# insitro/FastVim

Hardware: AMD Instinct MI355X
Metric: images/sec FastVim-T 224px bs=128/GPU fwd+bwd (+all-reduce +AdamW +EMA), whole job (higher is better)
Workload: dtype bf16; 1 GPU; FastVim-T 224x224 bs=128/GPU bf16 training step, synthetic ImageNet tensors (BASELINE configs[1]); global_batch=128, parallelism=dp1, hip_graph=True, optimizer_in_step=True, final_loss_hex=0x1.779ca20000000p+0

## Files before the change

fastvim_amd/_lib.py:

```python
import ctypes
import os
import threading

import torch

_PKG = os.path.dirname(os.path.abspath(__file__))
LIB_PATH = os.path.join(_PKG, "libfastvim_hip.so")

FV_F32, FV_BF16, FV_F16 = 0, 1, 2
_DTYPES = {torch.float32: FV_F32, torch.bfloat16: FV_BF16, torch.float16: FV_F16}

_lib = None

C_ABI_SYMBOLS = (
    "fv_last_error", "fv_version",
    "fv_selective_scan_fwd", "fv_selective_scan_bwd_workspace", "fv_selective_scan_bwd",
    "fv_causal_conv1d_fwd", "fv_causal_conv1d_bwd", "fv_scan_expand_skip_fwd",
    "fv_mixer_conv_pool_fwd", "fv_mixer_scan_fwd", "fv_mixer_xproj_scan_fwd_ok", "fv_mixer_xproj_scan_fwd", "fv_mixer_combine_fwd",
    "fv_mixer_bwd_blocks", "fv_mixer_combine_bwd", "fv_mixer_scan_bwd_chunks", "fv_mixer_scan_bwd_chunks_b",
    "fv_mixer_scan_bwd_ckpt_floats", "fv_mixer_scan_bwd_partials", "fv_mixer_scan_bwd", "fv_mixer_scan_bwd_dir", "fv_mixer_scan_bwd_ckpt", "fv_mixer_scan_bwd_segments", "fv_mixer_scan_bwd_seg_floats", "fv_mixer_scan_bwd_seg_partials", "fv_mixer_scan_bwd_seg_chunks", "fv_mixer_scan_bwd_seg", "fv_mixer_scan_fwd_ckpt", "fv_mixer_scan_ckpt_floats", "fv_mixer_scan_fwd_segments", "fv_mixer_scan_fwd_seg_floats", "fv_mixer_scan_fwd_seg", "fv_rows_segment_sum", "fv_rows_gather", "fv_mixer_conv_pool_bwd", "fv_mixer_conv_pool_bwd2_ok", "fv_mixer_conv_pool_bwd2", "fv_mixer_scan_bwd_xproj_ok", "fv_mixer_scan_bwd_xproj", "fv_chunk_rows_bf16", "fv_reduce_partials", "fv_reduce_partials_multi",
    "fv_add_norm_blocks", "fv_add_norm_fwd", "fv_add_norm_bwd", "fv_gemm_bf16", "fv_gemm_bf16_tn_grouped", "fv_gemm_bf16_tn_grouped_ld", "fv_mixer_xproj_fwd", "fv_mixer_xproj_bwd_slices", "fv_mixer_xproj_bwd", "fv_mixer_xproj_bwd2", "fv_mixer_xproj_bwd3_ok", "fv_mixer_xproj_bwd3", "fv_adamw_flat", "fv_soft_target_ce",
    "fv_patch_unfold", "fv_gemm_bf16_rowbias", "fv_mean_pool_fwd", "fv_mean_pool_bwd", "fv_droppath_table", "fv_scale_cast",
    "fv_column_sum", "fv_gemm_bf16_addnorm", "fv_gemm_bf16_dgrad_addnorm_blocks", "fv_gemm_bf16_dgrad_addnorm_bwd", "fv_gemm_bf16_dgrad_addnorm_bwd2", "fv_gemm_bf16_addnorm2", "fv_mixer_combine_out_proj_addnorm_ok", "fv_mixer_combine_out_proj_addnorm", "fv_gemm_f32",
    "fv_mixer_conv_pool_bwd_dgrad_ok", "fv_mixer_conv_pool_bwd_dgrad_blocks", "fv_mixer_conv_pool_bwd_dgrad", "fv_transpose_bf16_batched", "fv_gemm_bf16_tn_grouped_wide8",
# ... 5 lines not shown
    "fv_patch_unfold_chan", "fv_chan_embed_table", "fv_chan_embed_scatter",
    "fv_mixer_plan",
    "fv_bn1d_stats", "fv_bn1d_apply", "fv_bn1d_bwd", "fv_sgd_flat", "fv_lars_partials_per_segment", "fv_lars_sumsq_partials", "fv_lars_flat",
    "fv_tap_ln_blocks", "fv_tap_ln_fwd", "fv_tap_ln_bwd", "fv_ln2d_blocks", "fv_ln2d_fwd", "fv_ln2d_bwd",
    "fv_swap_params_ema", "fv_eval_accumulate",
    "fv_patch_unfold_u8", "fv_patch_unfold_mix_u8", "fv_patch_unfold_chan_u8",
    "fv_random_erase", "fv_patch_unfold_u8_re", "fv_patch_unfold_mix_u8_re",
    "fv_mae_loss_ok", "fv_mae_loss_fwd", "fv_mae_loss_bwd",
    "fv_mae_mask_plan", "fv_tokens_gather", "fv_mae_decoder_tokens_fwd", "fv_mae_decoder_tokens_bwd",
    "fv_resample_u8_ok", "fv_resample_workspace_ints", "fv_resample_coeffs", "fv_resample_u8",
    "fv_randaug_ok", "fv_randaug_workspace_bytes", "fv_randaug_stats", "fv_randaug_apply",
    "fv_jpeg_probe", "fv_jpeg_entropy_decode", "fv_jpeg_table_ints", "fv_jpeg_idct", "fv_jpeg_rgb",
    "fv_jpeg_packed_bound", "fv_jpeg_entropy_decode_packed", "fv_jpeg_idct_packed",
    "fv_mae_noise", "fv_mae_mask_plan_keyed",
    "fv_jpeg_index_bound", "fv_jpeg_build_index", "fv_jpeg_index_stage", "fv_jpeg_stream_table_ints", "fv_jpeg_huff",
)


_tls = threading.local()


class _DeviceGuarded:

    def __init__(self, cdll):
        self._cdll = cdll
        self._wrapped = {}

    def __getattr__(self, name):
        w = self._wrapped.get(name)
        if w is None:
# ... 73 lines not shown
```

fastvim_amd/csrc/gemm_mfma.hip:

```cpp
#include <stdlib.h>
#include <utility>

#include "common.h"
#include "gemm_tiles.h"

namespace {


#ifdef FASTVIM_TUNING_HOOKS
unsigned long long* g_fv_stamps = nullptr;
__device__ __forceinline__ void fv_stamp(unsigned long long* buf, int slot) {
  if (buf && threadIdx.x == 0) {
    unsigned long long t;
    __builtin_amdgcn_sched_barrier(0);
    asm volatile("s_memtime %0\n\ts_waitcnt lgkmcnt(0)" : "=s"(t)::"memory");
    __builtin_amdgcn_sched_barrier(0);
    buf[(size_t)blockIdx.x * 8 + slot] = t;
  }
}
#define FV_STAMP(ne, slot) fv_stamp((ne)->stamps, slot)
#else
#define FV_STAMP(ne, slot) ((void)0)
#endif

// ... 46 lines not shown
  const int tiles_n = (p.N + BN - 1) / BN, tiles_m = (p.M + BM - 1) / BM;
  const int nblk = NORM_EPI != 0 ? (int)gridDim.x : tiles_m * tiles_n;
  int bid = block_id;
  if constexpr (XREMAP) {
    const int q8 = nblk / 8, r8 = nblk % 8, xcd = bid % 8, j = bid / 8;
    bid = (xcd < r8 ? xcd * (q8 + 1) : r8 * (q8 + 1) + (xcd - r8) * q8) + j;
  }
  const int tm = bid / tiles_n, tn = bid % tiles_n;
  const int rpt = (NORM_EPI != 0 && ne->rpt > 0) ? ne->rpt : BM;
  const int m0 = tm * rpt, n0 = tn * BN;
  const int mlim = NORM_EPI != 0 ? min(p.M, m0 + rpt) : p.M;
  const int kbeg = split * p.k_per_split;
  const int kend = min(p.K, kbeg + p.k_per_split);
  const int nt = (kend - kbeg + BK - 1) / BK;

  if constexpr (NORM_EPI != 0) FV_STAMP(ne, 0);
  f32x4 acc[NB][MB];
#pragma unroll
  for (int a = 0; a < NB; ++a)
#pragma unroll
    for (int b = 0; b < MB; ++b) acc[a][b] = (f32x4){0.f, 0.f, 0.f, 0.f};
  constexpr bool NE_PRE = NORM_EPI != 0 && BM <= 64;
  constexpr int NE_IT = NE_PRE ? BM / 4 / 8 : 1;
  float4 ne_r[NE_IT][2][3];
  float4 ne_g[NORM_EPI == 2 ? NE_IT : 1][2][3];
  if constexpr (NORM_EPI == 2 && NE_PRE) {
    const int lr = lane % 16, gr = lane / 16;
#pragma unroll
    for (int it = 0; it < NE_IT; ++it)
#pragma unroll
      for (int u = 0; u < 2; ++u) {
        const int row = m0 + wv * (BM / 4) + it * 8 + u * 4 + gr, rowc = row < p.M ? row : p.M - 1;
#pragma unroll
        for (int k = 0; k < 3; ++k)
          ne_g[it][u][k] = ne->dres_out ? *reinterpret_cast<const float4*>(ne->dres_out + (size_t)rowc * BN + (k * 16 + lr) * 4)
                                        : make_float4(0.f, 0.f, 0.f, 0.f);
      }
  }
  if constexpr (NE_PRE) {
    const int lr = lane % 16, gr = lane / 16;
#pragma unroll
// ... 26 lines not shown
        if constexpr (OPA) fa[i] = ka.get(ks, i);
        else fa[i] = frag<AMODE, BM>(sA(cur), wm * MB + i, ks, lane);
      }
#pragma unroll
      for (int i = 0; i < NB; ++i) {
        if constexpr (OPB) fb[i] = kb.get(ks, i);
        else fb[i] = frag<BMODE, BN>(sB(cur), wn * NB + i, ks, lane);
      }
#pragma unroll
      for (int a = 0; a < NB; ++a)
#pragma unroll
        for (int b = 0; b < MB; ++b)
          acc[a][b] = __builtin_amdgcn_mfma_f32_16x16x32_bf16(fb[a], fa[b], acc[a][b], 0, 0, 0);
    }
  };
  if constexpr (GLDS) {
    GldsPlan<AMODE, BM, NT> ga;
    GldsPlan<BMODE, BN, NT> gb;
    ga.init(p.A, p.lda, m0, p.M, tid);
    gb.init(p.B, p.ldb, n0, p.N, tid);
    ga.issue(sA(0), kbeg, tid);
    gb.issue(sB(0), kbeg, tid);
    __syncthreads();
    if constexpr (NORM_EPI != 0) FV_STAMP(ne, 1);
    for (int t = 0; t < nt; ++t) {
      const int cur = t & 1;
#ifdef FASTVIM_TUNING_HOOKS
      if (t + 1 < nt && dbg != 2) {
        ga.issue(sA(cur ^ 1), kbeg + (dbg == 3 ? 0 : (t + 1) * BK), tid);
        gb.issue(sB(cur ^ 1), kbeg + (dbg == 3 ? 0 : (t + 1) * BK), tid);
      }
// ... 31 lines not shown
  }
  if constexpr (NORM_EPI != 0) FV_STAMP(ne, 2);
  const long zoff = (long)split * p.c_split_stride;
  if (p.bias && p.rb_period <= 0) {
#pragma unroll
    for (int a = 0; a < NB; ++a) {
      const int n = n0 + wn * WNC + a * 16 + (lane >> 4) * 4;
#pragma unroll
      for (int j = 0; j < 4; ++j) {
        const float bj = (n + j < p.N) ? p.bias[n + j] : 0.f;
#pragma unroll
        for (int b = 0; b < MB; ++b) acc[a][b][j] += bj;
      }
    }
  }
  if constexpr (NORM_EPI == 2) {
    static_assert(BN == 192 && WM * WN == 4 && BM % 32 == 0, "whole 192-wide rows, four waves");
    constexpr int RSB = BN * 2 + 16, LPR = 16, RPW = 4, RU = 2, RW = BM / 4;
    __syncthreads();
#pragma unroll
    for (int b = 0; b < MB; ++b)
#pragma unroll
      for (int a = 0; a < NB; ++a) {
        const f32x4 v = acc[a][b];
        uint2 pk = {pack_bf16x2(v[0], v[1]), pack_bf16x2(v[2], v[3])};
        *reinterpret_cast<uint2*>(smem + (wm * WMR + b * 16 + (lane & 15)) * RSB + (wn * WNC + a * 16 + (lane >> 4) * 4) * 2) = pk;
      }
    __syncthreads();
    FV_STAMP(ne, 3);
    const int lr = lane % LPR, gr = lane / LPR;
    const float inv_n = 1.f / (float)BN;
    float w[3][4], aw[3][4];
#pragma unroll
    for (int k = 0; k < 3; ++k) {
      const float4 t = *reinterpret_cast<const float4*>(ne->w + (k * LPR + lr) * 4);
      w[k][0] = t.x; w[k][1] = t.y; w[k][2] = t.z; w[k][3] = t.w;
#pragma unroll
      for (int e = 0; e < 4; ++e) aw[k][e] = 0.f;
    }
#pragma unroll
    for (int it = 0; it < RW / (RPW * RU); ++it) {
#pragma unroll
      for (int u = 0; u < RU; ++u) {
        const int rl = wv * RW + it * (RPW * RU) + u * RPW + gr;
        const int row = m0 + rl;
        const bool live = row < mlim;
        const int rowc = live ? row : p.M - 1;
        const size_t base = (size_t)rowc * BN;
        const float rstd = ne->rstd[rowc];
        const float sc = ne->row_scale ? ne->row_scale[rowc / ne->rows_per_scale] : 1.f;
        const float lv = live ? 1.f : 0.f;
        float xh[3][4], dxh[3][4];
        float c2 = 0.f;
#pragma unroll
        for (int k = 0; k < 3; ++k) {
          const int c = (k * LPR + lr) * 4;
          const uint2 xb = *reinterpret_cast<const uint2*>(smem + rl * RSB + c * 2);
          const float dyv[4] = {__uint_as_float(xb.x << 16), __uint_as_float(xb.x & 0xffff0000u),
                                __uint_as_float(xb.y << 16), __uint_as_float(xb.y & 0xffff0000u)};
          float4 rr4;
          if constexpr (NE_PRE) rr4 = ne_r[it][u][k];
          else rr4 = *reinterpret_cast<const float4*>(ne->residual + base + c);
          const float rr[4] = {rr4.x, rr4.y, rr4.z, rr4.w};
#pragma unroll
          for (int e = 0; e < 4; ++e) {
            const float dyl = dyv[e] * lv;
            xh[k][e] = (rr[e] - 0.f) * rstd;
            dxh[k][e] = dyl * w[k][e];
            aw[k][e] = fmaf(dyl, xh[k][e], aw[k][e]);
            c2 = fmaf(dxh[k][e], xh[k][e], c2);
          }
        }
#define FV_DPP_ADD(ctrl) c2 += __int_as_float(__builtin_amdgcn_update_dpp(0, __float_as_int(c2), ctrl, 0xf, 0xf, true))
        FV_DPP_ADD(0xB1);
        FV_DPP_ADD(0x4E);
        FV_DPP_ADD(0x141);
        FV_DPP_ADD(0x140);
#undef FV_DPP_ADD
        c2 = c2 * inv_n;
        const float c1 = 0.f;
#pragma unroll
        for (int k = 0; k < 3; ++k) {
          const int c = (k * LPR + lr) * 4;
          float4 g4;
// ... 9 lines not shown
#pragma unroll
              for (int e = 0; e < 4; ++e) dr[e] *= sc;
            uint2 pk = {pack_bf16x2(dr[0], dr[1]), pack_bf16x2(dr[2], dr[3])};
            *reinterpret_cast<uint2*>(ne->y + base + c) = pk;
            *reinterpret_cast<uint2*>(smem + rl * RSB + c * 2) = pk;
          } else {
            *reinterpret_cast<uint2*>(smem + rl * RSB + c * 2) = make_uint2(0u, 0u);
          }
        }
      }
    }
    __syncthreads();
    FV_STAMP(ne, 4);
    float* s_acc = reinterpret_cast<float*>(smem + BM * RSB);
#pragma unroll
    for (int k = 0; k < 3; ++k)
#pragma unroll
      for (int e = 0; e < 4; ++e) {
        float v = aw[k][e];
        auto r1 = __builtin_amdgcn_permlane16_swap(__float_as_uint(v), __float_as_uint(v), false, false);
        v = __uint_as_float(r1[0]) + __uint_as_float(r1[1]);
        auto r2 = __builtin_amdgcn_permlane32_swap(__float_as_uint(v), __float_as_uint(v), false, false);
        v = __uint_as_float(r2[0]) + __uint_as_float(r2[1]);
        if (gr == 0) s_acc[wv * BN + (k * LPR + lr) * 4 + e] = v;
      }
    __syncthreads();
    float* dst = ne->pw + (size_t)block_id * BN;
    for (int c = tid; c < BN; c += NT) dst[c] = (s_acc[c] + s_acc[BN + c]) + (s_acc[2 * BN + c] + s_acc[3 * BN + c]);
    FV_STAMP(ne, 5);
    if (ne->W2) {
      __syncthreads();
      constexpr int O_B = (BM * RSB + 255) / 256 * 256, O_S = O_B + 2 * 128 * BK * 2;
      tile_times_w2<BM, RSB, KS>(smem, smem + O_B, smem + O_S, ne->W2, ne->ldw2, ne->N2, ne->C2, m0, mlim, tid);
    }
    FV_STAMP(ne, 6);
    return;
  }
  if constexpr (NORM_EPI == 1) {
    static_assert(BN == 192 && WM * WN == 4 && BM % 32 == 0, "whole 192-wide rows, four waves");
    constexpr int RSB = BN * 2 + 16, LPR = 16, RPW = 4, RU = 2, RW = BM / 4;
    __syncthreads();
#pragma unroll
    for (int b = 0; b < MB; ++b)
// ... 148 lines not shown
}

template <int AMODE, int BMODE, int WM, int WN, bool GLDS, int NB = 4, int MB = 4>
__global__ __launch_bounds__(64 * WM * WN, 2) void gemm_bf16_kernel(GemmParams p) {
  gemm_bf16_body<AMODE, BMODE, WM, WN, GLDS, NB, MB>(p, blockIdx.x, blockIdx.z);
}

template <int BMROWS>
__global__ __launch_bounds__(256, 2) void gemm_addnorm_kernel(GemmParams p, NormEpi ne) {
  gemm_bf16_body<KC, KC, 2, 2, true, 6, BMROWS / 32, true, 1>(p, blockIdx.x, 0, &ne);
}

template <int BMROWS>
__global__ __launch_bounds__(256, 2) void gemm_dgrad_addnorm_bwd_kernel(GemmParams p, NormEpi ne) {
  gemm_bf16_body<KC, KS, 2, 2, true, 6, BMROWS / 32, true, 2>(p, blockIdx.x, 0, &ne);
}

template <int NV_>
__device__ __forceinline__ void wait_vmc() { asm volatile("s_waitcnt vmcnt(%0)" ::"n"(NV_) : "memory"); }
template <int OFF>
__device__ __forceinline__ u32x4 ds_read_b128_imm(uint32_t a) {
  u32x4 v;
  asm volatile("ds_read_b128 %0, %1 offset:%2" : "=v"(v) : "v"(a), "n"(OFF));
  return v;
}

template <int AMODE, int BMODE, bool CF32, bool PERSIST = false>
__device__ __forceinline__ void p256_body(const GemmParams& p, int bid, int split, char* smem, int bid_stride = 0,
                                          int bid_end = 0) {
  constexpr int HALF = 128 * BK * 2;
// ... 777 lines not shown
    constexpr size_t s1 = (size_t)2 * (BMR + 192) * BK * 2;
    constexpr size_t s2 = ((size_t)BMR * 400 + 255) / 256 * 256 + 2 * 128 * BK * 2 + 4 * 32 * 144;
    const size_t smem = s1 > s2 ? s1 : s2;
    static FvOncePerDevice attr_set;   
    if (attr_set.first()) {
      (void)hipFuncSetAttribute((const void*)gemm_dgrad_addnorm_bwd_kernel<BMR>, hipFuncAttributeMaxDynamicSharedMemorySize, (int)smem);
      (void)0;         
    }
    hipLaunchKernelGGL((gemm_dgrad_addnorm_bwd_kernel<BMR>), dim3(fv_cdiv(M, ne.rpt)), dim3(256), smem, (hipStream_t)stream, p, ne);
  };
  go(std::integral_constant<int, 64>{});
  FV_LAUNCH_CHECK();
  return FV_OK;
}

extern "C" int fv_gemm_bf16_tn_grouped_wide8(int M, int N, int Kd) {
  static const int wide8 = fv_tune("FASTVIM_WGRAD_WIDE8", 1);
  if (!wide8 || Kd < 50000) return 0;
  if (M % 256 == 0 && N % 192 == 0 && N % 256 != 0 && (long)M * N >= 1024 * 384) return 4;
  if (M % 192 == 0 && N % 256 == 0 && M % 256 != 0 && (long)M * N >= 384 * 768) return 5;
  return 0;
}

extern "C" int fv_gemm_bf16_tn_grouped(const void* const* x, const void* const* y, float* const* parts, const int* Kd,
                                       const int* M, const int* N, const int* splits, int count, fv_stream_t stream) {
  return fv_gemm_bf16_tn_grouped_ld(x, y, parts, Kd, M, N, nullptr, nullptr, splits, count, stream);
}

extern "C" int fv_gemm_bf16_tn_grouped_ld(const void* const* x, const void* const* y, float* const* parts,
                                          const int* Kd, const int* M, const int* N, const int* ldx, const int* ldy,
// ... 139 lines not shown
```

fastvim_amd/fastvim.py:

```python
import math
from functools import partial
from typing import Optional

import torch
import torch.nn as nn
import torch.nn.functional as F
from torch import Tensor

from .dense_ops import tap_layer_norm_nchw
from .layernorm import RMSNorm, layer_norm_fn, rms_norm_fn
from .linear_probe import is_probe_head, probe_head_forward
from . import glue_ops as G
from . import pixels
from . import mamba_simple_faster as msf
from .mamba_simple_faster import (ChainedBlockFn, LinearFn, Mamba, OutProjAddNormFn, _compute_dtype, _direct_grad, _shadow,
                                  linear_dgrad, linear_wgrad, out_proj_add_norm_ok)
from .mixer_ops import reduce_partials


class _EmbedEpilogueFn(torch.autograd.Function):

    @staticmethod
    def forward(ctx, lin, bias, pos):
        ctx.lin_dtype = lin.dtype
        ctx.has = (bias is not None, pos is not None)
        pb = bias.float() if bias is not None else None
        if pos is not None:
            pb = pos.float() if pb is None else pos.float() + pb
        if pb is None:
            return lin.float()
        return torch.add(pb, lin)
# ... 394 lines not shown
        return x, (H, W)

    def _chainable(self, hidden_states, lo, hi, inference_params, out_indices, carried=False):
        if inference_params is not None or out_indices is not None or hi - lo < (1 if carried else 2) or not hidden_states.is_cuda:
            return False
        if _compute_dtype(hidden_states) != torch.bfloat16 or self.embed_dim != 192:
            return False
        for blk in self.layers[lo:hi]:
            mx = blk.mixer
            if (type(blk) is not Block or type(mx) is not Mamba or not blk.fused_add_norm or not blk.residual_in_fp32
                    or not isinstance(blk.norm, RMSNorm) or blk.norm.bias is not None or mx.init_layer_scale is not None
                    or mx.out_proj.bias is not None or mx.out_proj.weight.shape[1] % 64 or mx.d_conv != 4 or mx.d_state != 16):
                return False
        return True

    def _run_layers_chained(self, hidden_states, residual, lo, hi, pend=None, close=True):
        cdt = _compute_dtype(hidden_states if pend is None else pend[0])
        pack = None
        for layer_idx in range(lo, hi):
            blk = self.layers[layer_idx]
            scale = None
            if residual is not None and isinstance(blk.drop_path, DropPath):
                scale = blk.drop_path.row_scale(hidden_states if pend is None else pend[0])
            rot = blk.rotate_every_block is True and blk.layer_idx % 2 != 0
            if pend is not None and out_proj_add_norm_ok(pend[0], pend[1], residual, blk.norm.weight, cdt):
                ChainedBlockFn.pending_in = pack
                ChainedBlockFn.defer = msf.COMBINE_IN_OUT_PROJ and torch._C._autograd._top_saved_tensors_default_hooks(True) is None
                ChainedBlockFn.pending_out = None
                try:
                    g, residual = ChainedBlockFn.apply(pend[0], pend[1], residual, blk.norm.weight, float(blk.norm.eps), scale,
                                                       *blk.mixer.mixer_fn_args(cdt, rot, defer_out_proj=True))
# ... 2 lines not shown
                    raise
                finally:
                    ChainedBlockFn.pending_in, ChainedBlockFn.defer = None, False
                pack, ChainedBlockFn.pending_out = ChainedBlockFn.pending_out, None
                pend = (g, blk.mixer.out_proj.weight)
                continue
            else:
                msf.resolve_combine(pack)
                pack = None
                if pend is not None:
                    hidden_states = LinearFn.apply(pend[0], pend[1], cdt)
                hidden_states, residual = layer_norm_fn(
                    hidden_states, blk.norm.weight, blk.norm.bias, residual=residual, eps=blk.norm.eps, prenorm=True,
                    residual_in_fp32=blk.residual_in_fp32, is_rms_norm=True, row_scale=scale, out_dtype=cdt)
            pend = (blk.mixer(hidden_states, transposed_grid=rot, defer_out_proj=True), blk.mixer.out_proj.weight)
        msf.resolve_combine(pack)
        if not close:
            return None, residual, pend
        return LinearFn.apply(pend[0], pend[1], cdt), residual

    def _run_layers_open(self, hidden_states, residual, lo, hi, pend=None):
        probe = hidden_states if pend is None else pend[0]
        if self._chainable(probe, lo, hi, None, None, carried=True):
            return self._run_layers_chained(hidden_states, residual, lo, hi, pend=pend, close=False)
        if pend is not None:
            hidden_states = self._close_run(pend)
        hidden_states, residual = self._run_layers(hidden_states, residual, lo, hi)
        return hidden_states, residual, None

    def _close_run(self, pend):
        return LinearFn.apply(pend[0], pend[1], _compute_dtype(pend[0]))

    def _run_layers(self, hidden_states, residual, lo, hi, inference_params=None, out_indices=None, outs=None):
        if self._chainable(hidden_states, lo, hi, inference_params, out_indices):
            return self._run_layers_chained(hidden_states, residual, lo, hi)
        for layer_idx in range(lo, hi):
            hidden_states, residual = self.layers[layer_idx](hidden_states, residual, inference_params=inference_params)
            if out_indices is not None and layer_idx in out_indices:
                outs.append(hidden_states)
        return hidden_states, residual

    def _final(self, hidden_states, residual):
        is_rms = isinstance(self.norm_f, RMSNorm)
        if not self.fused_add_norm:
            residual = hidden_states if residual is None else residual + self.drop_path(hidden_states)
            hidden_states = layer_norm_fn(residual.to(self.norm_f.weight.dtype), self.norm_f.weight, self.norm_f.bias,
# ... 15 lines not shown

    def _head(self, x):
        if isinstance(self.head, nn.Linear) and x.is_cuda:
            x = LinearFn.apply(x, self.head.weight, _compute_dtype(x), self.head.bias)
        elif is_probe_head(self.head) and x.is_cuda:
            x = probe_head_forward(self.head, x)
        else:
            x = self.head(x)
        if self.final_pool_type == "max":
            x = x.max(dim=1)[0]
        return x

    def forward_features(self, x, inference_params=None, out_indices=None):
        hidden_states, (H, W) = self._embed(x)
        outs = []
        hidden_states, residual = self._run_layers(hidden_states, None, 0, len(self.layers), inference_params,
                                                   out_indices, outs)
        if out_indices is not None:
            assert len(outs) == len(out_indices)
            return outs, (H, W)
        return self._final(hidden_states, residual)

    def forward(self, x, return_features=False, inference_params=None):
        half = msf.half_io(x) or self.pos_embed_dtype_is_half()
        x = self.forward_features(x, inference_params)
        if not return_features:
            x = self._head(x)
        return x.to(torch.float16) if half and torch.is_tensor(x) and x.is_floating_point() else x

    def pos_embed_dtype_is_half(self):
# ... 127 lines not shown
```

fastvim_amd/mamba_simple_faster.py:

```python
import ctypes
import math

import torch
import torch.nn as nn
import torch.nn.functional as F

from . import _lib as L
from . import mixer_ops as M
from .gemm import gemm_any_bnn, gemm_any_btn, gemm_any_nn, gemm_any_nt, gemm_any_tn, gemm_nn, gemm_nt, gemm_tn


def _shadow(w, cdt):
    sh = getattr(w, "_fv_shadow", None)
    if sh is not None and sh.dtype == cdt:
        if w._version != w._fv_shadow_version:
            with torch.no_grad():
                sh.copy_(w)
            w._fv_shadow_version = w._version
        return sh
    return w.to(cdt)


def _shadow_t(w, cdt):
    wt = getattr(w, "_fv_shadow_t", None)
# ... 278 lines not shown
                dw = M.reduce_partials(pw, nb).to(ctx.w_param.dtype)
            g2 = g.view(Mrows, d_in)
            dg = linear_dgrad(dx, _shadow(W_out, cdt)).view(B, Ltok, d_in)
            dW_out = _SideStream.run(lambda: linear_wgrad(dx, g2, W_out), dx, g)
        return dg, dW_out, dres_in.view(B, Ltok, d), dw, None, None, None


class _Ctx:

    def save_for_backward(self, *tensors):
        self.saved_tensors = tensors


COMBINE_IN_OUT_PROJ = True
CONV_IN_DGRAD = True
XPROJ_TWO_ADDENDS = True


def resolve_combine(pack):
    if pack is not None:
        M.combine_fwd(pack["xz"], pack["skip"], pack["yc"], pack["ln_w"], pack["ln_b"], pack["eps"], pack["rows"],
                      pack["cols"], pack["transposed"], out=pack["out"])


def _out_proj_add_norm_fwd(g, W_out, residual, norm_w, eps, row_scale, cdt, W_in=None, pack=None):
    B, Ltok, d_in = g.shape
    d = W_out.shape[0]
    Mrows = B * Ltok
    g2 = g.view(Mrows, d_in)
    res2 = residual.reshape(Mrows, d).contiguous()
# ... 126 lines not shown
            gd = _direct_grad(ctx.w_param)
            if gd is not None:
                M.reduce_partials(out["pw"], out["nb"], out=gd.view(-1), accumulate=True)
                dw = None
            else:
                dw = M.reduce_partials(out["pw"], out["nb"]).to(ctx.w_param.dtype)
            dx = out["dx"]
            d_in = g_prev.shape[2]
            g2 = g_prev.view(Mrows, d_in)
            dg_prev = out["dg_prev"] if out["dg_prev"] is not None else linear_dgrad(dx, _shadow(W_out_prev, cdt))
            dg_prev = dg_prev.view(B, Ltok, d_in)
            dW_out = _SideStream.run(lambda: linear_wgrad(dx, g2, W_out_prev), dx, g_prev)
        return (dg_prev, dW_out, out["dres_in"].view(B, Ltok, d), dw, None, None) + tuple(grads[1:1 + ctx.n_mixer_args])


def out_proj_add_norm_ok(g, W_out, residual, norm_w, cdt):
    return (g.is_cuda and cdt == torch.bfloat16 and g.dtype == torch.bfloat16 and g.is_contiguous()
            and W_out.shape[0] == 192 and W_out.shape[1] % 64 == 0 and residual is not None
            and residual.dtype == torch.float32 and norm_w.dtype == torch.float32)


def _compute_dtype(t):
    if torch.is_autocast_enabled():
        dt = torch.get_autocast_dtype('cuda')
        return torch.float32 if dt == torch.float16 else dt
    return torch.float32 if t.dtype == torch.float16 else t.dtype


def half_io(t):
    if torch.is_autocast_enabled():
# ... 298 lines not shown
```

fastvim_amd/mixer_ops.py:

```python
import ctypes

import torch

from . import _lib as L

f32 = ctypes.c_float


def _geo(rows, cols, transposed):
    return (1, rows) if transposed else (cols, 1)


def conv_pool_fwd(xz, conv_w, conv_b, conv_w_b, conv_b_b, rows, cols, transposed, pool_max, scaling, tpp=1,
                  D=None, D_b=None):
    B, Ltok, two_d = xz.shape
    d_in = two_d // 2
    s_i, s_j = _geo(rows, cols, transposed)
    xc = torch.empty(2, B, rows * tpp, d_in, device=xz.device, dtype=xz.dtype)
    skip = torch.empty(B, Ltok, d_in, device=xz.device, dtype=xz.dtype) if D is not None else None
    amax = torch.empty_like(xc) if pool_max else None
    rc = L.lib().fv_mixer_conv_pool_fwd(
        L.ptr(xz), L.ptr(conv_w), L.ptr(conv_b), L.ptr(conv_w_b), L.ptr(conv_b_b), L.ptr(D), L.ptr(D_b), L.ptr(xc),
        L.ptr(skip), L.ptr(amax), L.i32(B), L.i32(rows), L.i32(cols), L.i32(s_i), L.i32(s_j), L.i32(tpp), L.i32(d_in),
        L.i32(conv_w.shape[-1]), L.i32(pool_max), f32(scaling), L.i32(L.dtype_code(xz.dtype)), L.stream_of(xz))
# ... 143 lines not shown
    n = part.numel() // n_partials
    assert out.numel() == n and out.is_contiguous() and out.dtype == torch.float32
    rc = L.lib().fv_reduce_partials(L.ptr(part), L.ptr(out), L.i32(n_partials), ctypes.c_size_t(n),
                                    L.i32(accumulate), L.stream_of(part))
    L.check(rc, "reduce_partials")
    return out


def combine_out_proj_addnorm_ok(xz, rows, cols, tpp, d_model):
    B, Ltok, two_d = xz.shape
    return bool(xz.dtype == torch.bfloat16 and xz.is_contiguous() and
                L.lib().fv_mixer_combine_out_proj_addnorm_ok(L.i32(B), L.i32(rows), L.i32(cols), L.i32(tpp), L.i32(two_d // 2),
                                                             L.i32(d_model), L.i32(L.FV_BF16)))


def combine_out_proj_addnorm(xz, skip, yc, ln_w, ln_b, ln_eps, rows, cols, transposed, out, W_out_c, residual2, norm_w32,
                             row_scale, rows_per_scale, eps, W_out_pk=None):
    B, Ltok, two_d = xz.shape
    d = W_out_c.shape[0]
    Mrows = B * Ltok
    s_i, s_j = _geo(rows, cols, transposed)
    g, mean, rstd_ln = out
    y = torch.empty(Mrows, d, device=xz.device, dtype=torch.bfloat16)
    res_out = torch.empty(Mrows, d, device=xz.device, dtype=torch.float32)
    rstd = torch.empty(Mrows, device=xz.device, dtype=torch.float32)
    if W_out_pk is not None:
        assert W_out_pk.dtype == torch.bfloat16 and W_out_pk.is_contiguous() and W_out_pk.numel() == d * (two_d // 2)
        fn, W_arg, ldw = L.lib().fv_mixer_combine_out_proj_addnorm_pk, W_out_pk, two_d // 2
    else:
        fn, W_arg, ldw = L.lib().fv_mixer_combine_out_proj_addnorm, W_out_c, W_out_c.stride(0)
    rc = fn(
        L.ptr(xz), L.ptr(skip), L.ptr(yc), L.ptr(ln_w), L.ptr(ln_b), f32(ln_eps), L.ptr(g), L.ptr(mean), L.ptr(rstd_ln),
# ... 169 lines not shown
    rc = fn(
        L.ptr(xz), L.ptr(d_o), L.ptr(dxc), L.ptr(dxc2), L.ptr(conv_w), L.ptr(conv_b), L.ptr(conv_w_b), L.ptr(conv_b_b),
        L.ptr(D), L.ptr(D_b), L.ptr(dxz), L.ptr(part), L.i32(B), L.i32(rows), L.i32(cols), L.i32(s_i), L.i32(s_j),
        f32(scaling), L.ptr(W_arg), ctypes.c_long(ldwt), L.ptr(dres_out), L.ptr(r), L.ptr(rstd), L.ptr(norm_w32),
        L.ptr(row_scale), L.i32(rows_per_scale), L.ptr(dx), L.ptr(dres_in), L.ptr(pw), L.ptr(W2_arg), L.ptr(dg_prev), L.i32(N2),
        ctypes.c_long(ldw2), L.stream_of(xz))
    L.check(rc, "mixer_conv_pool_bwd_dgrad")
    if conv_grad_out is not None:
        reduce_partials(part, nb, out=conv_grad_out, accumulate=True)
        p2 = None
    else:
        p2 = reduce_partials(part, nb)
    return p2, dx, dres_in, pw, nb, dg_prev


def transpose_bf16_batched(srcs, dsts):
    lib = L.lib()
    rows, cols = srcs[0].shape
    for lo in range(0, len(srcs), 64):
        a, b = srcs[lo:lo + 64], dsts[lo:lo + 64]
        assert all(t.dtype == torch.bfloat16 and t.is_contiguous() and tuple(t.shape) == (rows, cols) for t in a)
        assert all(t.dtype == torch.bfloat16 and t.is_contiguous() and tuple(t.shape) == (cols, rows) for t in b)
        k = len(a)
        ins = (ctypes.c_void_p * k)(*[t.data_ptr() for t in a])
        outs = (ctypes.c_void_p * k)(*[t.data_ptr() for t in b])
        L.check(lib.fv_transpose_bf16_batched(ins, outs, L.i32(k), L.i32(rows), L.i32(cols), L.stream_of(a[0])), "transpose_bf16_batched")


PACK_ROWS = 192

# ... 198 lines not shown
```

include/fastvim_hip.h:

```cpp
#ifndef FASTVIM_HIP_H
#define FASTVIM_HIP_H

#include <stddef.h>
#include <stdint.h>

#ifdef __cplusplus
extern "C" {
#endif

typedef void* fv_stream_t;

enum { FV_F32 = 0, FV_BF16 = 1, FV_F16 = 2 };
enum { FV_OK = 0, FV_ERR_INVALID = -1, FV_ERR_HIP = -2, FV_ERR_UNSUPPORTED = -3 };

const char* fv_last_error(void);
#define FV_ABI_VERSION 3
int fv_version(void);

int fv_selective_scan_fwd(const void* u, const void* delta, const float* A, const void* B,
                          const void* C, const float* D, const void* z, const float* delta_bias,
                          void* out, float* last_state, int batch, int dim, int seqlen, int dstate,
                          int n_groups, int B_variable, int C_variable, int delta_softplus,
                          int dtype, fv_stream_t stream);

// ... 152 lines not shown
int fv_gemm_bf16_addnorm(const void* A, const void* W, const float* residual, const float* norm_weight,
                         const float* row_scale, int rows_per_scale, void* y, float* residual_out, float* rstd, int M,
                         int N, int K, long lda, long ldw, float eps, fv_stream_t stream);

int fv_gemm_bf16_dgrad_addnorm_blocks(int M);
int fv_gemm_bf16_dgrad_addnorm_bwd(const void* A, const void* W, const float* dresidual_out, const float* r,
                                   const float* rstd, const float* norm_weight, const float* row_scale,
                                   int rows_per_scale, void* dx, float* dresidual_in, float* partial_dw, int M, int N,
                                   int K, long lda, long ldw, fv_stream_t stream);

int fv_gemm_bf16_dgrad_addnorm_bwd2(const void* A, const void* W, const float* dresidual_out, const float* r,
                                    const float* rstd, const float* norm_weight, const float* row_scale,
                                    int rows_per_scale, void* dx, float* dresidual_in, float* partial_dw, int M, int N,
                                    int K, long lda, long ldw, const void* W2, void* C2, int N2, long ldw2,
                                    fv_stream_t stream);

int fv_mixer_combine_out_proj_addnorm_ok(int batch, int rows, int cols, int tokens_per_patch, int d_inner, int d_model,
                                         int dtype);
int fv_mixer_combine_out_proj_addnorm(const void* xz, const void* skip, const float* yc, const float* ln_w,
                                      const float* ln_b, float ln_eps, void* g, float* mean, float* rstd_ln, int batch,
                                      int rows, int cols, int tok_stride_row, int tok_stride_col, const void* W, long ldw,
                                      const float* residual, const float* norm_weight, const float* row_scale,
                                      int rows_per_scale, void* y, float* residual_out, float* rstd, float eps,
                                      fv_stream_t stream);
int fv_mixer_combine_out_proj_addnorm_pk(const void* xz, const void* skip, const float* yc, const float* ln_w,
                                         const float* ln_b, float ln_eps, void* g, float* mean, float* rstd_ln, int batch,
                                         int rows, int cols, int tok_stride_row, int tok_stride_col, const void* W,
                                         long ldw, const float* residual, const float* norm_weight,
                                         const float* row_scale, int rows_per_scale, void* y, float* residual_out,
                                         float* rstd, float eps, fv_stream_t stream);
// ... 286 lines not shown
```

Before: 25700 images/sec.

## Fuse final norm and mean-pool backward into the last block's out-proj dgrad kernel

Adds a ChainCloseFn that closes the last chained Mamba layer together with the final RMSNorm and mean pool. In backward, a new kernel variant (NORM_EPI==3) skips the GEMM mainloop, broadcasts the pooled gradient divided by the token count directly into shared memory, then runs the existing add-norm backward epilogue and the fused W2 dgrad. This removes the separate mean-pool backward, the final norm backward and the materialised broadcast gradient. Partial norm-weight sums are packed per 32-row slot so the existing reduce_partials still works. The cost is a more complex templated epilogue and a new path that only applies to this configuration.

```diff
diff --git a/fastvim_amd/_lib.py b/fastvim_amd/_lib.py
--- a/fastvim_amd/_lib.py
+++ b/fastvim_amd/_lib.py
@@ -43,6 +43,7 @@
     "fv_jpeg_packed_bound", "fv_jpeg_entropy_decode_packed", "fv_jpeg_idct_packed",
     "fv_mae_noise", "fv_mae_mask_plan_keyed",
     "fv_jpeg_index_bound", "fv_jpeg_build_index", "fv_jpeg_index_stage", "fv_jpeg_stream_table_ints", "fv_jpeg_huff",
+    "fv_pool_addnorm_bwd_dgrad",
 )
 
 
diff --git a/fastvim_amd/csrc/gemm_mfma.hip b/fastvim_amd/csrc/gemm_mfma.hip
--- a/fastvim_amd/csrc/gemm_mfma.hip
+++ b/fastvim_amd/csrc/gemm_mfma.hip
@@ -84,6 +84,8 @@
   const int kend = min(p.K, kbeg + p.k_per_split);
   const int nt = (kend - kbeg + BK - 1) / BK;
 
+  constexpr bool ADJ = NORM_EPI == 2 || NORM_EPI == 3;
+  constexpr bool POOL = NORM_EPI == 3;
   if constexpr (NORM_EPI != 0) FV_STAMP(ne, 0);
   f32x4 acc[NB][MB];
 #pragma unroll
@@ -93,8 +95,8 @@
   constexpr bool NE_PRE = NORM_EPI != 0 && BM <= 64;
   constexpr int NE_IT = NE_PRE ? BM / 4 / 8 : 1;
   float4 ne_r[NE_IT][2][3];
-  float4 ne_g[NORM_EPI == 2 ? NE_IT : 1][2][3];
-  if constexpr (NORM_EPI == 2 && NE_PRE) {
+  float4 ne_g[ADJ ? NE_IT : 1][2][3];
+  if constexpr (ADJ && NE_PRE) {
     const int lr = lane % 16, gr = lane / 16;
 #pragma unroll
     for (int it = 0; it < NE_IT; ++it)
@@ -151,7 +153,8 @@
           acc[a][b] = __builtin_amdgcn_mfma_f32_16x16x32_bf16(fb[a], fa[b], acc[a][b], 0, 0, 0);
     }
   };
-  if constexpr (GLDS) {
+  if constexpr (POOL) {
+  } else if constexpr (GLDS) {
     GldsPlan<AMODE, BM, NT> ga;
     GldsPlan<BMODE, BN, NT> gb;
     ga.init(p.A, p.lda, m0, p.M, tid);
@@ -213,10 +216,24 @@
       }
     }
   }
-  if constexpr (NORM_EPI == 2) {
+  if constexpr (ADJ) {
     static_assert(BN == 192 && WM * WN == 4 && BM % 32 == 0, "whole 192-wide rows, four waves");
     constexpr int RSB = BN * 2 + 16, LPR = 16, RPW = 4, RU = 2, RW = BM / 4;
     __syncthreads();
+    if constexpr (POOL) {
+      constexpr int CPR = BN / 8;
+      const float inv = ne->eps;
+      for (int e = tid; e < BM * CPR; e += NT) {
+        const int rl = e / CPR, c = e - rl * CPR;
+        const int row = min(m0 + rl, p.M - 1);
+        const u32x4 g = *reinterpret_cast<const u32x4*>(p.A + (size_t)(row / p.K) * BN + c * 8);
+        u32x4 o;
+#pragma unroll
+        for (int q = 0; q < 4; ++q)
+          o[q] = pack_bf16x2(__uint_as_float(g[q] << 16) * inv, __uint_as_float(g[q] & 0xffff0000u) * inv);
+        *reinterpret_cast<u32x4*>(smem + rl * RSB + c * 16) = o;
+      }
+    } else {
 #pragma unroll
     for (int b = 0; b < MB; ++b)
 #pragma unroll
@@ -225,17 +242,21 @@
         uint2 pk = {pack_bf16x2(v[0], v[1]), pack_bf16x2(v[2], v[3])};
         *reinterpret_cast<uint2*>(smem + (wm * WMR + b * 16 + (lane & 15)) * RSB + (wn * WNC + a * 16 + (lane >> 4) * 4) * 2) = pk;
       }
+    }
     __syncthreads();
     FV_STAMP(ne, 3);
     const int lr = lane % LPR, gr = lane / LPR;
     const float inv_n = 1.f / (float)BN;
-    float w[3][4], aw[3][4];
+    constexpr int NAW = POOL ? RW / (RPW * RU) : 1;
+    float w[3][4], aw[NAW][3][4];
 #pragma unroll
     for (int k = 0; k < 3; ++k) {
       const float4 t = *reinterpret_cast<const float4*>(ne->w + (k * LPR + lr) * 4);
       w[k][0] = t.x; w[k][1] = t.y; w[k][2] = t.z; w[k][3] = t.w;
 #pragma unroll
-      for (int e = 0; e < 4; ++e) aw[k][e] = 0.f;
+      for (int a = 0; a < NAW; ++a)
+#pragma unroll
+        for (int e = 0; e < 4; ++e) aw[a][k][e] = 0.f;
     }
 #pragma unroll
     for (int it = 0; it < RW / (RPW * RU); ++it) {
@@ -266,7 +287,7 @@
             const float dyl = dyv[e] * lv;
             xh[k][e] = (rr[e] - 0.f) * rstd;
             dxh[k][e] = dyl * w[k][e];
-            aw[k][e] = fmaf(dyl, xh[k][e], aw[k][e]);
+            aw[POOL ? it : 0][k][e] = fmaf(dyl, xh[k][e], aw[POOL ? it : 0][k][e]);
             c2 = fmaf(dxh[k][e], xh[k][e], c2);
           }
         }
@@ -306,19 +327,34 @@
     FV_STAMP(ne, 4);
     float* s_acc = reinterpret_cast<float*>(smem + BM * RSB);
 #pragma unroll
+    for (int a = 0; a < NAW; ++a)
+#pragma unroll
     for (int k = 0; k < 3; ++k)
 #pragma unroll
       for (int e = 0; e < 4; ++e) {
-        float v = aw[k][e];
+        float v = aw[a][k][e];
         auto r1 = __builtin_amdgcn_permlane16_swap(__float_as_uint(v), __float_as_uint(v), false, false);
         v = __uint_as_float(r1[0]) + __uint_as_float(r1[1]);
         auto r2 = __builtin_amdgcn_permlane32_swap(__float_as_uint(v), __float_as_uint(v), false, false);
         v = __uint_as_float(r2[0]) + __uint_as_float(r2[1]);
-        if (gr == 0) s_acc[wv * BN + (k * LPR + lr) * 4 + e] = v;
+        if (gr == 0) s_acc[(wv * NAW + a) * BN + (k * LPR + lr) * 4 + e] = v;
       }
     __syncthreads();
+    if constexpr (POOL) {
+      static_assert(BM == 64 && NAW == 2, "two 32-row partial rows per tile");
+      const int nrows = p.k_per_split, ntiles = (int)gridDim.x;
+      for (int j = 0; j < 2; ++j)
+        if (2 * tm + j < nrows) {
+          float* dst = ne->pw + (size_t)(2 * tm + j) * BN;
+          const float* s = s_acc + 4 * j * BN;
+          for (int c = tid; c < BN; c += NT) dst[c] = (s[c] + s[BN + c]) + (s[2 * BN + c] + s[3 * BN + c]);
+        }
+      for (int z = 2 * ntiles + tm; z < nrows; z += ntiles)
+        for (int c = tid; c < BN; c += NT) ne->pw[(size_t)z * BN + c] = 0.f;
+    } else {
     float* dst = ne->pw + (size_t)block_id * BN;
     for (int c = tid; c < BN; c += NT) dst[c] = (s_acc[c] + s_acc[BN + c]) + (s_acc[2 * BN + c] + s_acc[3 * BN + c]);
+    }
     FV_STAMP(ne, 5);
     if (ne->W2) {
       __syncthreads();
@@ -497,6 +533,11 @@
 template <int BMROWS>
 __global__ __launch_bounds__(256, 2) void gemm_dgrad_addnorm_bwd_kernel(GemmParams p, NormEpi ne) {
   gemm_bf16_body<KC, KS, 2, 2, true, 6, BMROWS / 32, true, 2>(p, blockIdx.x, 0, &ne);
+}
+
+template <int BMROWS>
+__global__ __launch_bounds__(256, 2) void pool_addnorm_bwd_dgrad_kernel(GemmParams p, NormEpi ne) {
+  gemm_bf16_body<KC, KS, 2, 2, true, 6, BMROWS / 32, true, 3>(p, blockIdx.x, 0, &ne);
 }
 
 template <int NV_>
@@ -1304,6 +1345,40 @@
   return FV_OK;
 }
 
+extern "C" int fv_pool_addnorm_bwd_dgrad(const void* d_pooled, int batch, int tokens, const float* r, const float* rstd,
+                                         const float* norm_weight, const float* row_scale, int rows_per_scale, void* dx,
+                                         float* dresidual_in, float* partial_dw, const void* W2, void* C2, int N2, long ldw2,
+                                         fv_stream_t stream) {
+  FV_CHECK(d_pooled && r && rstd && norm_weight && dx && dresidual_in && partial_dw, "pool_addnorm_bwd_dgrad: null pointer");
+  FV_CHECK(batch > 0 && tokens > 0 && (long)batch * tokens < (1L << 31), "pool_addnorm_bwd_dgrad: bad shape (%d, %d)", batch, tokens);
+  FV_CHECK(((uintptr_t)d_pooled & 15) == 0 && ((uintptr_t)r & 15) == 0 && ((uintptr_t)dresidual_in & 15) == 0 && ((uintptr_t)dx & 7) == 0,
+           "pool_addnorm_bwd_dgrad: operands must be 16-byte aligned");
+  FV_CHECK(!row_scale || rows_per_scale > 0, "pool_addnorm_bwd_dgrad: rows_per_scale must be positive");
+  if (W2) {
+    FV_CHECK(C2 && N2 > 0 && N2 % 128 == 0 && ldw2 >= N2 && ldw2 % 8 == 0 && ((uintptr_t)W2 & 15) == 0 && ((uintptr_t)C2 & 15) == 0,
+             "pool_addnorm_bwd_dgrad: the second weight must be (192, N2) with N2 a multiple of 128, 16-byte aligned");
+  }
+  const int M = batch * tokens, N = 192;
+  const int nrows = fv_add_norm_blocks(M);
+  if ((long)nrows * 32 < M) return FV_ERR_UNSUPPORTED;
+  GemmParams p{};
+  p.A = (const bf16_t*)d_pooled; p.C = dx;
+  p.M = M; p.N = N; p.K = tokens; p.ldc = N; p.k_per_split = nrows;
+  NormEpi ne{r, norm_weight, row_scale, dresidual_in, (bf16_t*)dx, const_cast<float*>(rstd),
+             rows_per_scale > 0 ? rows_per_scale : 1, 1.f / (float)tokens, nullptr, partial_dw,
+             (const bf16_t*)W2, (bf16_t*)C2, ldw2, N2, 64};
+#ifdef FASTVIM_TUNING_HOOKS
+  ne.stamps = g_fv_stamps;
+#endif
+  constexpr size_t smem = ((size_t)64 * 400 + 255) / 256 * 256 + 2 * 128 * BK * 2 + 4 * 32 * 144;
+  static FvOncePerDevice attr_set;
+  if (attr_set.first())
+    (void)hipFuncSetAttribute((const void*)pool_addnorm_bwd_dgrad_kernel<64>, hipFuncAttributeMaxDynamicSharedMemorySize, (int)smem);
+  hipLaunchKernelGGL((pool_addnorm_bwd_dgrad_kernel<64>), dim3(fv_cdiv(M, ne.rpt)), dim3(256), smem, (hipStream_t)stream, p, ne);
+  FV_LAUNCH_CHECK();
+  return FV_OK;
+}
+
 extern "C" int fv_gemm_bf16_tn_grouped_wide8(int M, int N, int Kd) {
   static const int wide8 = fv_tune("FASTVIM_WGRAD_WIDE8", 1);
   if (!wide8 || Kd < 50000) return 0;
diff --git a/fastvim_amd/fastvim.py b/fastvim_amd/fastvim.py
--- a/fastvim_amd/fastvim.py
+++ b/fastvim_amd/fastvim.py
@@ -13,8 +13,8 @@
 from . import glue_ops as G
 from . import pixels
 from . import mamba_simple_faster as msf
-from .mamba_simple_faster import (ChainedBlockFn, LinearFn, Mamba, OutProjAddNormFn, _compute_dtype, _direct_grad, _shadow,
-                                  linear_dgrad, linear_wgrad, out_proj_add_norm_ok)
+from .mamba_simple_faster import (ChainCloseFn, ChainedBlockFn, LinearFn, Mamba, OutProjAddNormFn,
+                                  _compute_dtype, _direct_grad, _shadow, linear_dgrad, linear_wgrad, out_proj_add_norm_ok)
 from .mixer_ops import reduce_partials
 
 
@@ -439,7 +439,7 @@
                 return False
         return True
 
-    def _run_layers_chained(self, hidden_states, residual, lo, hi, pend=None, close=True):
+    def _run_layers_chained(self, hidden_states, residual, lo, hi, pend=None, close=True, final=False):
         cdt = _compute_dtype(hidden_states if pend is None else pend[0])
         pack = None
         for layer_idx in range(lo, hi):
@@ -472,10 +472,23 @@
                     hidden_states, blk.norm.weight, blk.norm.bias, residual=residual, eps=blk.norm.eps, prenorm=True,
                     residual_in_fp32=blk.residual_in_fp32, is_rms_norm=True, row_scale=scale, out_dtype=cdt)
             pend = (blk.mixer(hidden_states, transposed_grid=rot, defer_out_proj=True), blk.mixer.out_proj.weight)
+        if final and pend is not None and self._close_in_chain_ok(pend, residual, cdt):
+            scale = self.drop_path.row_scale(pend[0]) if isinstance(self.drop_path, DropPath) else None
+            ChainCloseFn.pending_in = pack
+            try:
+                return ChainCloseFn.apply(pend[0], pend[1], residual, self.norm_f.weight, float(self.norm_f.eps), scale, cdt)
+            finally:
+                ChainCloseFn.pending_in = None
         msf.resolve_combine(pack)
         if not close:
             return None, residual, pend
-        return LinearFn.apply(pend[0], pend[1], cdt), residual
+        hidden_states = LinearFn.apply(pend[0], pend[1], cdt)
+        return self._final(hidden_states, residual) if final else (hidden_states, residual)
+
+    def _close_in_chain_ok(self, pend, residual, cdt):
+        return (self.fused_add_norm and self.final_pool_type == "mean" and self.residual_in_fp32
+                and isinstance(self.norm_f, RMSNorm) and self.norm_f.bias is None
+                and msf.chain_close_ok(pend[0], pend[1], residual, self.norm_f.weight, cdt))
 
     def _run_layers_open(self, hidden_states, residual, lo, hi, pend=None):
         probe = hidden_states if pend is None else pend[0]
@@ -488,6 +501,12 @@
 
     def _close_run(self, pend):
         return LinearFn.apply(pend[0], pend[1], _compute_dtype(pend[0]))
+
+    def _run_layers_final(self, hidden_states, residual, lo, hi):
+        if self._chainable(hidden_states, lo, hi, None, None):
+            return self._run_layers_chained(hidden_states, residual, lo, hi, final=True)
+        hidden_states, residual = self._run_layers(hidden_states, residual, lo, hi)
+        return self._final(hidden_states, residual)
 
     def _run_layers(self, hidden_states, residual, lo, hi, inference_params=None, out_indices=None, outs=None):
         if self._chainable(hidden_states, lo, hi, inference_params, out_indices):
@@ -533,6 +552,8 @@
     def forward_features(self, x, inference_params=None, out_indices=None):
         hidden_states, (H, W) = self._embed(x)
         outs = []
+        if out_indices is None and inference_params is None:
+            return self._run_layers_final(hidden_states, None, 0, len(self.layers))
         hidden_states, residual = self._run_layers(hidden_states, None, 0, len(self.layers), inference_params,
                                                    out_indices, outs)
         if out_indices is not None:
diff --git a/fastvim_amd/mamba_simple_faster.py b/fastvim_amd/mamba_simple_faster.py
--- a/fastvim_amd/mamba_simple_faster.py
+++ b/fastvim_amd/mamba_simple_faster.py
@@ -316,6 +316,7 @@
 
 COMBINE_IN_OUT_PROJ = True
 CONV_IN_DGRAD = True
+CLOSE_IN_CHAIN = True
 XPROJ_TWO_ADDENDS = True
 
 
@@ -472,6 +473,67 @@
         return (dg_prev, dW_out, out["dres_in"].view(B, Ltok, d), dw, None, None) + tuple(grads[1:1 + ctx.n_mixer_args])
 
 
+class ChainCloseFn(torch.autograd.Function):
+
+    pending_in = None
+
+    @staticmethod
+    def forward(ctx, g_prev, W_out_prev, residual, norm_w, eps, row_scale, cdt):
+        from .glue_ops import MeanPoolFn
+        L.require_gpu(g_prev, W_out_prev, residual, norm_w)
+        B, Ltok, _ = g_prev.shape
+        d = W_out_prev.shape[0]
+        pack, ChainCloseFn.pending_in = ChainCloseFn.pending_in, None
+        assert pack is None or pack["out"][0].data_ptr() == g_prev.data_ptr()
+        with torch.autocast("cuda", enabled=False):
+            W_out_c = _shadow(W_out_prev, cdt)
+            if pack is not None and W_out_c.stride(1) == 1 and W_out_c.stride(0) % 8 == 0 and W_out_c.data_ptr() % 16 == 0:
+                w32 = norm_w.float().contiguous()
+                rs = row_scale.float().contiguous() if row_scale is not None else None
+                rps = B * Ltok // rs.numel() if rs is not None else 1
+                pooled, res_out, rstd = M.combine_out_proj_addnorm_pool(
+                    pack["xz"], pack["skip"], pack["yc"], pack["ln_w"], pack["ln_b"], pack["eps"], pack["rows"], pack["cols"],
+                    pack["transposed"], pack["out"], W_out_c, residual.reshape(B * Ltok, d).contiguous(), w32, rs, rps, eps,
+                    W_out_pk=_shadow_pk(W_out_prev, cdt, W_out_c))
+            else:
+                y, res_out, rstd, w32, rs, rps = _out_proj_add_norm_fwd(g_prev, W_out_prev, residual, norm_w, eps, row_scale,
+                                                                      cdt, pack=pack)
+                pooled = MeanPoolFn.forward(_Ctx(), y.view(B, Ltok, d))
+        ctx.save_for_backward(g_prev, W_out_prev, res_out, w32, rstd, rs)
+        ctx.rows_per_scale = rps
+        ctx.cdt = cdt
+        ctx.shape = (B, Ltok, d)
+        ctx.w_param = norm_w
+        return pooled
+
+    @staticmethod
+    def backward(ctx, dpooled):
+        g_prev, W_out_prev, r, w32, rstd, row_scale = ctx.saved_tensors
+        B, Ltok, d = ctx.shape
+        Mrows, cdt, d_in = B * Ltok, ctx.cdt, g_prev.shape[2]
+        with torch.autocast("cuda", enabled=False):
+            W2 = _shadow(W_out_prev, cdt)
+            dx, dres_in, pw, nb, dg_prev = M.pool_addnorm_bwd_dgrad(
+                dpooled.to(cdt).contiguous(), Ltok, r, rstd, w32, row_scale, ctx.rows_per_scale,
+                W2=W2 if d_in % 128 == 0 else None)
+            gd = _direct_grad(ctx.w_param)
+            if gd is not None:
+                M.reduce_partials(pw, nb, out=gd.view(-1), accumulate=True)
+                dw = None
+            else:
+                dw = M.reduce_partials(pw, nb).to(ctx.w_param.dtype)
+            if dg_prev is None:
+                dg_prev = linear_dgrad(dx, W2)
+            g2 = g_prev.view(Mrows, d_in)
+            dW_out = _SideStream.run(lambda: linear_wgrad(dx, g2, W_out_prev), dx, g_prev)
+        return dg_prev.view(B, Ltok, d_in), dW_out, dres_in.view(B, Ltok, d), dw, None, None, None
+
+
+def chain_close_ok(g, W_out, residual, norm_w, cdt):
+    return (CLOSE_IN_CHAIN and out_proj_add_norm_ok(g, W_out, residual, norm_w, cdt) and W_out.is_contiguous()
+            and M.pool_addnorm_bwd_dgrad_ok(g.shape[0] * g.shape[1]))
+
+
 def out_proj_add_norm_ok(g, W_out, residual, norm_w, cdt):
     return (g.is_cuda and cdt == torch.bfloat16 and g.dtype == torch.bfloat16 and g.is_contiguous()
             and W_out.shape[0] == 192 and W_out.shape[1] % 64 == 0 and residual is not None
diff --git a/fastvim_amd/mixer_ops.py b/fastvim_amd/mixer_ops.py
--- a/fastvim_amd/mixer_ops.py
+++ b/fastvim_amd/mixer_ops.py
@@ -181,8 +181,27 @@
                                                              L.i32(d_model), L.i32(L.FV_BF16)))
 
 
+def combine_out_proj_addnorm_pool(xz, skip, yc, ln_w, ln_b, ln_eps, rows, cols, transposed, out, W_out_c, residual2, norm_w32,
+                                  row_scale, rows_per_scale, eps, W_out_pk=None):
+    B, Ltok, _ = xz.shape
+    y, res_out, rstd = _combine_out_proj_addnorm(xz, skip, yc, ln_w, ln_b, ln_eps, rows, cols, transposed, out, W_out_c, residual2,
+                                                 norm_w32, row_scale, rows_per_scale, eps, W_out_pk)
+    d = y.shape[1]
+    pooled = torch.empty(B, d, device=y.device, dtype=y.dtype)
+    rc = L.lib().fv_mean_pool_fwd(L.ptr(y), L.ptr(pooled), L.i32(B), L.i32(Ltok), L.i32(d), L.i32(L.dtype_code(y.dtype)),
+                                  L.stream_of(y))
+    L.check(rc, "mean_pool_fwd")
+    return pooled, res_out, rstd
+
+
 def combine_out_proj_addnorm(xz, skip, yc, ln_w, ln_b, ln_eps, rows, cols, transposed, out, W_out_c, residual2, norm_w32,
                              row_scale, rows_per_scale, eps, W_out_pk=None):
+    return _combine_out_proj_addnorm(xz, skip, yc, ln_w, ln_b, ln_eps, rows, cols, transposed, out, W_out_c, residual2, norm_w32,
+                                     row_scale, rows_per_scale, eps, W_out_pk)
+
+
+def _combine_out_proj_addnorm(xz, skip, yc, ln_w, ln_b, ln_eps, rows, cols, transposed, out, W_out_c, residual2, norm_w32,
+                              row_scale, rows_per_scale, eps, W_out_pk=None):
     B, Ltok, two_d = xz.shape
     d = W_out_c.shape[0]
     Mrows = B * Ltok
@@ -382,6 +401,31 @@
     return p2, dx, dres_in, pw, nb, dg_prev
 
 
+def pool_addnorm_bwd_dgrad_ok(Mrows):
+    return 32 * L.lib().fv_add_norm_blocks(L.i32(Mrows)) >= Mrows
+
+
+def pool_addnorm_bwd_dgrad(d_pooled, Ltok, r, rstd, norm_w32, row_scale, rows_per_scale, W2=None):
+    B, d = d_pooled.shape
+    Mrows = B * Ltok
+    assert d == 192 and d_pooled.dtype == torch.bfloat16 and d_pooled.is_contiguous()
+    assert r.dtype == torch.float32 and r.is_contiguous() and r.numel() == Mrows * d and rstd.numel() == Mrows
+    lib = L.lib()
+    dev = d_pooled.device
+    nb = lib.fv_add_norm_blocks(L.i32(Mrows))
+    dx = torch.empty(Mrows, d, device=dev, dtype=torch.bfloat16)
+    dres_in = torch.empty(Mrows, d, device=dev, dtype=torch.float32)
+    pw = torch.empty(nb, d, device=dev, dtype=torch.float32)
+    N2 = W2.shape[1] if W2 is not None else 0
+    dg_prev = torch.empty(Mrows, N2, device=dev, dtype=torch.bfloat16) if W2 is not None else None
+    rc = lib.fv_pool_addnorm_bwd_dgrad(
+        L.ptr(d_pooled), L.i32(B), L.i32(Ltok), L.ptr(r), L.ptr(rstd), L.ptr(norm_w32), L.ptr(row_scale),
+        L.i32(rows_per_scale), L.ptr(dx), L.ptr(dres_in), L.ptr(pw), L.ptr(W2), L.ptr(dg_prev), L.i32(N2),
+        ctypes.c_long(W2.stride(0) if W2 is not None else 0), L.stream_of(d_pooled))
+    L.check(rc, "pool_addnorm_bwd_dgrad")
+    return dx, dres_in, pw, nb, dg_prev
+
+
 def transpose_bf16_batched(srcs, dsts):
     lib = L.lib()
     rows, cols = srcs[0].shape
diff --git a/include/fastvim_hip.h b/include/fastvim_hip.h
--- a/include/fastvim_hip.h
+++ b/include/fastvim_hip.h
@@ -190,6 +190,11 @@
                                     int rows_per_scale, void* dx, float* dresidual_in, float* partial_dw, int M, int N,
                                     int K, long lda, long ldw, const void* W2, void* C2, int N2, long ldw2,
                                     fv_stream_t stream);
+
+int fv_pool_addnorm_bwd_dgrad(const void* d_pooled, int batch, int tokens, const float* r, const float* rstd,
+                              const float* norm_weight, const float* row_scale, int rows_per_scale, void* dx,
+                              float* dresidual_in, float* partial_dw, const void* W2, void* C2, int N2, long ldw2,
+                              fv_stream_t stream);
 
 int fv_mixer_combine_out_proj_addnorm_ok(int batch, int rows, int cols, int tokens_per_patch, int d_inner, int d_model,
                                          int dtype);
```

After: 25840 images/sec, median of 6. No clear change (+0.6%).
